# stockeh/swift

Hardware: AMD Instinct MI355X
Metric: 6h forecast steps/sec (members x ICs) on 128x256x69 ERA5 (higher is better)
Workload: dtype bf16

## Files before the change

### swift_amd/csrc/gemm.hip

```cpp
#include "common.h"

int g_persist_wgs = 256;

namespace {

template <typename OutT>
__device__ __forceinline__ float swiglu_out(float g, float u) {
    if constexpr (sizeof(OutT) == 4) return g / (1.0f + expf(-g)) * u;
    else return g * __builtin_amdgcn_rcpf(1.0f + __expf(-g)) * u;
}

constexpr int BM = 256;
constexpr int BN = 352;
constexpr int ROWB = 128;
constexpr int A_BYTES = BM * ROWB;
constexpr int B_BYTES = BN * ROWB;
constexpr int STAGE = A_BYTES + B_BYTES;
constexpr int LDS_BYTES = 2 * STAGE;
constexpr int NT = 512;
constexpr int A_PIECES = A_BYTES / 1024;
constexpr int B_PIECES = B_BYTES / 1024;
constexpr int MI = 4, NI = 11;

constexpr int EPI_QKNORM_TILED = 4;
// ... 241 lines not shown
    const int r16 = lane & 15;
    const int xoff = (wm * 64 + r16) * ROWB;
    const int woff = A_BYTES + (wn * 176 + r16) * ROWB;
    const int ch0 = (((lane >> 4) + 0) ^ (r16 >> 1)) * 16;
    const int ch1 = (((lane >> 4) + 4) ^ (r16 >> 1)) * 16;

    auto compute = [&](const char* s) {
#pragma unroll
        for (int ks = 0; ks < 2; ++ks) {
            const int ch = ks ? ch1 : ch0;
            uint4 xf[MI];
#pragma unroll
            for (int i = 0; i < MI; ++i) xf[i] = *reinterpret_cast<const uint4*>(s + xoff + i * 16 * ROWB + ch);
#pragma unroll
            for (int j = 0; j < NI; ++j) {
                const uint4 wf = *reinterpret_cast<const uint4*>(s + woff + j * 16 * ROWB + ch);
#pragma unroll
                for (int i = 0; i < MI; ++i) mma_chunk<T>(acc[i][j], wf, xf[i]);
            }
        }
    };

    const int nk = g.K / (ROWB / (int)sizeof(T));
    stage_load(stage0, 0);
    for (int kt = 0; kt < nk; kt += 2) {
        __builtin_amdgcn_s_waitcnt(0x0F70);
        __syncthreads();
        if (kt + 1 < nk) stage_load(stage1, kt + 1);
        compute(stage0);
        if (kt + 1 < nk) {
            __builtin_amdgcn_s_waitcnt(0x0F70);
            __syncthreads();
            if (kt + 2 < nk) stage_load(stage0, kt + 2);
            compute(stage1);
        }
    }

    if constexpr (EPI == SWIFTK_EPI_QKNORM || EPI == EPI_QKNORM_TILED)
        qknorm_tile<NI>(acc, lane, n0 + wn * 176, g.ep0, const_cast<float*>(g.ep1), m0 + wm * 64, g.M, g.N / 88);
    OutT* C = reinterpret_cast<OutT*>(g.C);
#pragma unroll
    for (int i = 0; i < MI; ++i) {
        const int m = m0 + wm * 64 + i * 16 + r16;
        if (m >= g.M) continue;
#pragma unroll
        for (int j = 0; j < NI; ++j) {
            const int nb = n0 + wn * 176 + j * 16 + 4 * (lane >> 4);
            if (nb >= g.N) continue;
            f32x4 v = acc[i][j];
            if constexpr (EPI == SWIFTK_EPI_BIAS_POS) {
                const float4 b = *reinterpret_cast<const float4*>(g.ep0 + nb);
                v[0] += b.x; v[1] += b.y; v[2] += b.z; v[3] += b.w;
                if (g.ep1) {
                    const float4 p = *reinterpret_cast<const float4*>(g.ep1 + (int64_t)(m % g.pos_rows) * g.N + nb);
                    v[0] += p.x; v[1] += p.y; v[2] += p.z; v[3] += p.w;
                }
            }
            if constexpr (EPI == SWIFTK_EPI_SWIGLU) {
                const float h0 = swiglu_out<OutT>(v[0], v[1]);
                const float h1 = swiglu_out<OutT>(v[2], v[3]);
                store2<OutT>(C + (int64_t)m * g.ldc + (nb >> 1), h0, h1);
            } else {
                store4<OutT>(C + (int64_t)m * g.ldc + nb, v[0], v[1], v[2], v[3]);
            }
        }
    }
}


struct TileIter {
    int ntm, ntn, gm;
    __device__ __forceinline__ void coords(int t, int& tm, int& tn) const {
        const int per = gm * ntn;
        const int grp = t / per, r = t - grp * per;
        const int rows = min(gm, ntm - grp * gm);
        tn = r / rows;
        tm = grp * gm + (r - tn * rows);
    }
};

template <typename T, typename OutT, int EPI, int NI, bool PPK, int SL = 0>
__global__ __launch_bounds__(NT) void gemm_kernel_p(GemmArgs g, int ntm, int gm) {
    constexpr bool SLE = (SL & 1) != 0, SLW = (SL & 2) != 0;
    static_assert(SL == 0 || (sizeof(T) == 2 && sizeof(OutT) == 2 && PPK && (EPI == SWIFTK_EPI_NONE || EPI == SWIFTK_EPI_SWIGLU)),
                  "the straight-line forms exist for the bf16 plain and SwiGLU epilogues of the ping-pong kernel only");
    constexpr int WT = 16 * NI;
    constexpr int BN = 2 * WT;
    constexpr int B_BYTES = BN * ROWB;
    constexpr int STAGE = A_BYTES + B_BYTES;
    constexpr int WP = B_BYTES / 1024;
    constexpr int HD = 8 * NI;
    constexpr bool PAIRED = EPI == SWIFTK_EPI_QKNORM_JVP || EPI == SWIFTK_EPI_SWIGLU_JVP;
    constexpr bool PP = PPK && sizeof(T) == 2;
    __shared__ __attribute__((aligned(16))) char smem[2 * STAGE];
    const int lane = threadIdx.x & 63;
    const int wv = __builtin_amdgcn_readfirstlane(threadIdx.x >> 6);
    const int wm = wv >> 1, wn = wv & 1;
    const TileIter it{ntm, g.ntn, gm};
    constexpr bool TAIL = EPI == EPI_NONE_TAIL;
    const int ksplit = TAIL || SLW ? 1 : g.ksplit;
    const int tail_from = TAIL ? g.tail_from : 0;
    const int ntiles = TAIL ? 2 * ntm * g.ntn - tail_from : ntm * g.ntn * ksplit;
    auto tile_of = [&](int item) {
        if constexpr (TAIL) return item < tail_from ? item : tail_from + ((item - tail_from) >> 1);
        else return item / ksplit;
    };
    auto split_of = [&](int item) {
        if constexpr (TAIL) return item < tail_from ? 0 : (item - tail_from) & 1;
        else return item % ksplit;
    };
    int vid;
    {
        const int nwg = gridDim.x, bid = blockIdx.x;
        const int q = nwg >> 3, r = nwg & 7, xcd = bid & 7;
        vid = (xcd < r ? xcd * (q + 1) : r * (q + 1) + (xcd - r) * q) + (bid >> 3);
    }
    const int stride = gridDim.x;
    if (vid >= ntiles) return;
    const uint32_t lds0 = (uint32_t)(uintptr_t)LDS_PTR(smem);

    const int prow = lane >> 3, pchunk = lane & 7;
    const uint32_t va_even = (uint32_t)(prow * g.lda_b) + 16u * (pchunk ^ ((prow >> 1) & 7));
    const uint32_t va_odd = (uint32_t)(prow * g.lda_b) + 16u * (pchunk ^ ((4 + (prow >> 1)) & 7));
    const uint32_t vb = (uint32_t)(prow * g.ldw_b) + 16u * (pchunk ^ ((4 * (wv & 1) + (prow >> 1)) & 7));
    [[maybe_unused]] const int tr2 = min(256 + wv * ((BN - 256 + 7) / 8) + min(lane, (BN - 256 + 7) / 8 - 1), BN - 1);
    [[maybe_unused]] int t_n0 = 0;
    const int nk_all = g.K / (ROWB / (int)sizeof(T));
    auto k_begin = [&](int item) {
        if constexpr (TAIL) return item >= tail_from && ((item - tail_from) & 1) ? nk_all >> 1 : 0;
        else return (int)((int64_t)(item % ksplit) * nk_all / ksplit);
    };
    auto k_end = [&](int item) {
        if constexpr (TAIL) return item >= tail_from && !((item - tail_from) & 1) ? nk_all >> 1 : nk_all;
        else return (int)((int64_t)(item % ksplit + 1) * nk_all / ksplit);
    };
    int tile = vid, kt = k_begin(vid);
    int w_grp = 0, w_tn = 0, w_rr = 0, s_grp = 0, s_tn = 0, s_rr = 0, n_tm = 0, n_tn = 0, c_tm = 0, c_tn = 0;
    if constexpr (SLW) {
        const int per = gm * g.ntn;
        w_grp = vid / per;
        int r = vid - w_grp * per;
        w_tn = r / gm;
        w_rr = r - w_tn * gm;
        s_grp = stride / per;
        r = stride - s_grp * per;
        s_tn = r / gm;
        s_rr = r - s_tn * gm;
    }
    auto walk_coords = [&](int& tm, int& tn) {
        const int rows = ntm - w_grp * gm;
        tm = w_grp * gm + w_rr;
        tn = w_tn;
        if (rows < gm) {
            const int r = w_tn * gm + w_rr;
            tn = r / rows;
            tm = w_grp * gm + (r - tn * rows);
        }
    };
    auto walk_step = [&] {
        w_rr += s_rr;
        int c = w_rr >= gm;
        w_rr -= c ? gm : 0;
        w_tn += s_tn + c;
        c = w_tn >= g.ntn;
        w_tn -= c ? g.ntn : 0;
        w_grp += s_grp + c;
    };
    auto src_coords = [&](int t, int& tm, int& tn) {
        if constexpr (SLW) { tm = n_tm; tn = n_tn; }
        else it.coords(tile_of(t), tm, tn);
    };
    const char* abase[4];
    const char* wbase[6];
    auto set_sources = [&](int t) {
        int tm, tn;
        it.coords(tile_of(t), tm, tn);
        t_n0 = tn * BN;
#pragma unroll
        for (int p = 0; p < 4; ++p) {
            int rb = tm * BM + (wv * 4 + p) * 8;
            if constexpr (PAIRED)
                rb = ((wv & 1) ? (g.M >> 1) : 0) + tm * (BM / 2) + (wv >> 1) * 32 + (p >> 1) * 16 + (p & 1) * 8;
            rb = rb < g.M ? rb : g.M - 8;
            abase[p] = g.A + (int64_t)rb * g.lda_b;
        }
#pragma unroll
        for (int i = 0; i < 6; ++i) {
            int rb = tn * BN + (wv + 8 * i) * 8;
            rb = rb < g.N ? rb : g.N - 8;
            if constexpr (sizeof(T) == 4 && EPI == SWIFTK_EPI_QKNORM)
                if (g.qk_only) rb += (rb / (2 * HD)) * HD;
            wbase[i] = g.W + (int64_t)rb * g.ldw_b;
        }
    };
    constexpr int JA = NI / 2, JB = NI - JA, JM = JA > JB ? JA : JB;
    const char* w0base[3];
    const char* w1base[3];
    auto w0row = [&](int i) { const int n = wv + 8 * i, h = n >= 2 * JA; return h * WT + (n - 2 * JA * h) * 8; };
    auto w1row = [&](int i) { const int n = wv + 8 * i, h = n >= 2 * JB; return h * WT + JA * 16 + (n - 2 * JB * h) * 8; };
    auto set_sources_aw1 = [&](int t) {
        int tm, tn;
        src_coords(t, tm, tn);
#pragma unroll
        for (int p = 0; p < 4; ++p) {
            int rb = tm * BM + (wv * 4 + p) * 8;
            if constexpr (PAIRED) rb = ((wv & 1) ? (g.M >> 1) : 0) + tm * (BM / 2) + (wv >> 1) * 32 + (p >> 1) * 16 + (p & 1) * 8;
            rb = rb < g.M ? rb : g.M - 8;
            abase[p] = g.A + (int64_t)rb * g.lda_b;
        }
#pragma unroll
        for (int i = 0; i < 3; ++i) {
            int rb = tn * BN + w1row(i);
            rb = rb < g.N ? rb : g.N - 8;
            w1base[i] = g.W + (int64_t)rb * g.ldw_b;
        }
    };
    auto set_sources_w0 = [&](int t) {
        int tm, tn;
        src_coords(t, tm, tn);
#pragma unroll
        for (int i = 0; i < 3; ++i) {
            int rb = tn * BN + w0row(i);
            rb = rb < g.N ? rb : g.N - 8;
            w0base[i] = g.W + (int64_t)rb * g.ldw_b;
        }
    };
    auto pp_a = [&](uint32_t sa, uint32_t koff, int p) {
        dma_piece_fast(sa + (wv * 4 + p) * 1024, abase[p], ((p & 1) ? va_odd : va_even) + koff);
    };
    auto pp_w0 = [&](uint32_t sa, uint32_t koff, int i) {
        if (wv + 8 * i < 4 * JA) dma_piece_fast(sa + A_BYTES + w0row(i) * ROWB, w0base[i], vb + koff);
    };
    auto pp_w1 = [&](uint32_t sa, uint32_t koff, int i) {
        if (wv + 8 * i < 4 * JB) dma_piece_fast(sa + A_BYTES + w1row(i) * ROWB, w1base[i], vb + koff);
    };
    auto issue_piece = [&](uint32_t sa, uint32_t koff, int p) {
        if (p < 4) {
            dma_piece_fast(sa + (wv * 4 + p) * 1024, abase[p], ((p & 1) ? va_odd : va_even) + koff);
        } else {
            const int i = p - 4;
            if (wv + 8 * i < WP) dma_piece_fast(sa + A_BYTES + (wv + 8 * i) * 1024, wbase[i], vb + koff);
        }
    };

    f32x4 acc[MI][NI];
#pragma unroll
    for (int i = 0; i < MI; ++i)
#pragma unroll
        for (int j = 0; j < NI; ++j) acc[i][j] = f32x4{0.f, 0.f, 0.f, 0.f};

    const int r16 = lane & 15;
    const int xoff = (wm * 64 + r16) * ROWB;
    const int woff = A_BYTES + (wn * WT + r16) * ROWB;
    const int ch0 = (((lane >> 4) + 0) ^ (r16 >> 1)) * 16;
    const int ch1 = (((lane >> 4) + 4) ^ (r16 >> 1)) * 16;

    int nk = k_end(tile);
    if constexpr (PP) {
        if constexpr (SLW) walk_coords(n_tm, n_tn);
        set_sources_aw1(tile);
        set_sources_w0(tile);
#pragma unroll
        for (int p = 0; p < 4; ++p) pp_a(lds0, (uint32_t)kt * ROWB, p);
#pragma unroll
        for (int i = 0; i < 3; ++i) pp_w0(lds0, (uint32_t)kt * ROWB, i);
#pragma unroll
        for (int i = 0; i < 3; ++i) pp_w1(lds0, (uint32_t)kt * ROWB, i);
    } else {
        set_sources(tile);
#pragma unroll
        for (int p = 0; p < 10; ++p) issue_piece(lds0, (uint32_t)kt * ROWB, p);
    }
    int par = 0;
    bool have_part = false;
    if (g.stagger != 0) {
        const int ph = g.stagger > 0 ? (((vid % gm) + (vid / gm)) & 7) : (int)(blockIdx.x & 7);
        const uint64_t t0 = __builtin_amdgcn_s_memrealtime();
        const uint64_t wait = (uint64_t)ph * (uint64_t)(g.stagger > 0 ? g.stagger : -g.stagger);
        while (__builtin_amdgcn_s_memrealtime() - t0 < wait) __builtin_amdgcn_s_sleep(16);
    }
    if (!PP && wv >= 4) __builtin_amdgcn_s_setprio(1);
    asm volatile("s_waitcnt vmcnt(0)" ::: "memory");
    const int grp = wv >> 2;
    bool first_kt = true;
#if SWIFTK_PP_STAMP
    unsigned long long* plog = nullptr;
    int pl_tile = 0, pl_kt = 0, pl_i = 0;
    if ((g.dbg & 64) && (wv & 3) == 0 && lane == 0 && (blockIdx.x & 31) == 0)
        plog = reinterpret_cast<unsigned long long*>(const_cast<float*>(g.ep1)) + ((blockIdx.x >> 5) * 2 + (wv >> 2)) * 20 * 16;
#define PP_STAMP() do { if (plog && pl_tile == 1 && pl_i < 16) plog[pl_kt * 16 + pl_i++] = __builtin_amdgcn_s_memtime(); } while (0)
#else
#define PP_STAMP() do {} while (0)
#endif
    for (;;) {
        if constexpr (PP) {
            if (first_kt) {
                __builtin_amdgcn_s_barrier();
                if (grp) __builtin_amdgcn_s_barrier();
            }
        } else {
            __builtin_amdgcn_s_barrier();
        }
        const char* s = smem + par * STAGE;
        const uint32_t fill = lds0 + (par ^ 1) * STAGE;
        const bool last_k = (kt + 1 == nk);
        const bool half = g.khalf && (kt + 1 == nk_all);
        uint32_t koff = (uint32_t)(kt + 1) * ROWB;
        if constexpr (PP) {
            const int ntile = tile + stride < ntiles ? tile + stride : tile;
            if (last_k) {
                if constexpr (SLW) {
                    walk_coords(c_tm, c_tn);
                    if (ntile != tile) walk_step();
                    walk_coords(n_tm, n_tn);
                }
                set_sources_aw1(ntile);
                set_sources_w0(ntile);
                koff = (uint32_t)k_begin(ntile) * ROWB;
            }
        } else
        if (last_k) {
            const int ntile = tile + stride;
            if (ntile < ntiles) set_sources(ntile);
            koff = (uint32_t)k_begin(ntile < ntiles ? ntile : tile) * ROWB;
// ... 286 lines not shown
                            const int j = jh + jj;
                            const int nb = n0 + wn * WT + j * 16 + 4 * g4;
                            const f32x4 v = acc[i][j];
                            acc[i][j] = f32x4{0.f, 0.f, 0.f, 0.f};
                            const uint4 hq = hb[gidx & 1][jj];
                            const uint32_t hw[4] = {hq.x, hq.y, hq.z, hq.w};
                            uint32_t o[4];
#pragma unroll
                            for (int e = 0; e < 4; ++e) {
                                const float gt = __uint_as_float(hw[e] << 16), up = __uint_as_float(hw[e] & 0xffff0000u);
                                const float sg = __builtin_amdgcn_rcpf(1.0f + __expf(-gt));
                                o[e] = pack_bf16(v[e] * up * (sg + gt * sg * (1.0f - sg)), v[e] * gt * sg);
                            }
                            if (m < g.M && nb < g.N)
                                *reinterpret_cast<uint4*>(C + (int64_t)m * g.ldc + 2 * nb) = make_uint4(o[0], o[1], o[2], o[3]);
                        }
                    }
                }
            } else
            if constexpr (EPI == SWIFTK_EPI_SWIGLU_BOTH) {
                constexpr int RS1 = WT * 2 + 16, RS2 = WT + 16;
                constexpr int CP1 = WT / 8, CP2 = WT / 16;
                __builtin_amdgcn_s_barrier();
                interior = (m0 + BM <= g.M) && (n0 + BN <= g.N);
                char* slab = const_cast<char*>(s) + wv * (16 * RS1);
                int elane = lane;
                asm volatile("" : "+v"(elane));
                const int g4 = elane >> 4;
                const int r16 = elane & 15;
                bf16_t* C2 = reinterpret_cast<bf16_t*>(const_cast<float*>(g.ep1));
                const int64_t ldc2 = g.pos_rows;
#pragma unroll
                for (int i = 0; i < MI; ++i) {
                    const int mrow0 = m0 + wm * 64 + i * 16;
#pragma unroll
                    for (int j = 0; j < NI; ++j) {
                        const f32x4 v = acc[i][j];
                        *reinterpret_cast<uint2*>(slab + r16 * RS1 + (j * 16 + 4 * g4) * 2) =
                            make_uint2(pack_bf16(v[0], v[1]), pack_bf16(v[2], v[3]));
                    }
                    __builtin_amdgcn_wave_barrier();
#pragma unroll
                    for (int t = 0; t < (16 * CP1 + 63) / 64; ++t) {
                        const int c = elane + 64 * t;
                        const int row = c / CP1, cc = c - row * CP1;
                        if (c < 16 * CP1) {
                            const uint4 q = *reinterpret_cast<const uint4*>(slab + row * RS1 + cc * 16);
                            const int m = mrow0 + row, n = n0 + wn * WT + cc * 8;
                            if (m < g.M && n < g.N) *reinterpret_cast<uint4*>(C + (int64_t)m * g.ldc + n) = q;
                        }
                    }
                    __builtin_amdgcn_wave_barrier();
#pragma unroll
                    for (int j = 0; j < NI; ++j) {
                        const f32x4 v = acc[i][j];
                        acc[i][j] = f32x4{0.f, 0.f, 0.f, 0.f};
                        const float h0 = v[0] * __builtin_amdgcn_rcpf(1.0f + __expf(-v[0])) * v[1];
                        const float h1 = v[2] * __builtin_amdgcn_rcpf(1.0f + __expf(-v[2])) * v[3];
                        *reinterpret_cast<uint32_t*>(slab + r16 * RS2 + (j * 8 + 2 * g4) * 2) = pack_bf16(h0, h1);
                    }
                    __builtin_amdgcn_wave_barrier();
#pragma unroll
                    for (int t = 0; t < (16 * CP2 + 63) / 64; ++t) {
                        const int c = elane + 64 * t;
                        const int row = c / CP2, cc = c - row * CP2;
                        if (c < 16 * CP2) {
                            const uint4 q = *reinterpret_cast<const uint4*>(slab + row * RS2 + cc * 16);
                            const int m = mrow0 + row, n = (n0 >> 1) + wn * (WT / 2) + cc * 8;
                            if (m < g.M && n < (g.N >> 1)) *reinterpret_cast<uint4*>(C2 + (int64_t)m * ldc2 + n) = q;
                        }
                    }
                    __builtin_amdgcn_wave_barrier();
                }
            } else
            if constexpr (sizeof(OutT) == 2 && EPI != SWIFTK_EPI_BIAS_POS) {
                constexpr bool SPLIT3 = EPI == SWIFTK_EPI_SWIGLU_SPLIT3;
                constexpr bool PAIROUT = EPI == EPI_BIAS_POS_PAIR;
                constexpr bool GLU = EPI == SWIFTK_EPI_SWIGLU || SPLIT3;
                constexpr int COLS = GLU ? WT / 2 : WT;
                constexpr int CPR = COLS / 8;
                constexpr int RSTR = COLS * 2 + 16;
                __builtin_amdgcn_s_barrier();
                interior = (m0 + BM <= g.M) && (n0 + BN <= g.N);
                char* slab = const_cast<char*>(s) + wv * (16 * RSTR);
                int elane = lane;
                asm volatile("" : "+v"(elane));
                const int g4 = elane >> 4;
                const int r16 = elane & 15;
                const int ncol0 = (GLU ? (n0 >> 1) : n0) + wn * COLS;
                const int nout = GLU ? (g.N >> 1) : g.N;
                uint32_t lo_pk[SPLIT3 || PAIROUT ? NI : 1];
                bool sl_done = false;
                if constexpr (SLE) {
                    if (interior) {
                        int el = lane;
                        asm volatile("" : "+v"(el));
                        const int sr16 = el & 15, sg4 = (el >> 4) & 3, l64 = el & 63;
                        constexpr int NCH = (16 * CPR + 63) / 64;
                        constexpr bool PART = (16 * CPR) % 64 != 0;
                        char* wr = slab + sr16 * RSTR + sg4 * (GLU ? 4 : 8);
                        const uint32_t ldcb = (uint32_t)g.ldc * 2u;
                        uint32_t ro[NCH], go[NCH];
#pragma unroll
                        for (int t = 0; t < NCH; ++t) {
                            const int c = l64 + 64 * t;
                            const int row = c / CPR, cc = c - row * CPR;
                            ro[t] = (uint32_t)(row * RSTR + cc * 16);
                            go[t] = (uint32_t)row * ldcb + (uint32_t)(cc * 16);
                        }
                        const bool part_on = l64 + 64 * (NCH - 1) < 16 * CPR;
                        char* cb = reinterpret_cast<char*>(C) + ((int64_t)(m0 + wm * 64) * g.ldc + ncol0) * 2;
#pragma unroll
                        for (int i = 0; i < MI; ++i) {
#pragma unroll
                            for (int j = 0; j < NI; ++j) {
                                const f32x4 v = acc[i][j];
                                acc[i][j] = f32x4{0.f, 0.f, 0.f, 0.f};
                                if constexpr (GLU) {
                                    const float h0 = v[0] * __builtin_amdgcn_rcpf(1.0f + __expf(-v[0])) * v[1];
                                    const float h1 = v[2] * __builtin_amdgcn_rcpf(1.0f + __expf(-v[2])) * v[3];
                                    *reinterpret_cast<uint32_t*>(wr + j * 16) = pack_bf16(h0, h1);
                                } else {
                                    *reinterpret_cast<uint2*>(wr + j * 32) = make_uint2(pack_bf16(v[0], v[1]), pack_bf16(v[2], v[3]));
                                }
                            }
                            __builtin_amdgcn_wave_barrier();
                            uint4 q[NCH];
#pragma unroll
                            for (int t = 0; t < NCH; ++t) q[t] = *reinterpret_cast<const uint4*>(slab + ro[t]);
#pragma unroll
                            for (int t = 0; t < NCH; ++t) {
                                if (!PART || t + 1 < NCH || part_on) store16_out_sbase(cb, go[t], q[t]);
                            }
                            __builtin_amdgcn_wave_barrier();
                            cb += (int64_t)g.ldc * 32;
                        }
                        sl_done = true;
                    }
                }
                if (!sl_done)
#pragma unroll
                for (int ii = 0; ii < MI; ++ii) {
                    const int i = EPI == SWIFTK_EPI_QKNORM_JVP ? ((ii & 1) ? ii >> 1 : 2 + (ii >> 1)) : ii;
#pragma unroll
                    for (int j = 0; j < NI; ++j) {
                        f32x4 v = acc[i][j];
                        if constexpr (EPI == SWIFTK_EPI_QKNORM_JVP) {
                            const bool first = 16 * j + 12 < 8 * NI ? true : (16 * j >= 8 * NI ? false : 16 * j + 4 * g4 < 8 * NI);
                            const float f = first ? qf[i & 1][0] : qf[i & 1][1];
                            if (i >= 2) {
                                const float fc = first ? qf[i & 1][2] : qf[i & 1][3];
                                const f32x4 pv = acc[i & 1][j];
#pragma unroll
                                for (int e = 0; e < 4; ++e) v[e] = fmaf(-fc, pv[e], f * v[e]);
                            } else {
                                v *= f;
                            }
                        }
                        acc[i][j] = f32x4{0.f, 0.f, 0.f, 0.f};
                        if constexpr (PAIROUT) {
                            const int nb = n0 + wn * WT + j * 16 + 4 * g4;
                            const int m = m0 + wm * 64 + i * 16 + r16;
                            if (m < g.M && nb < g.N) {
                                const float4 b = *reinterpret_cast<const float4*>(g.ep0 + nb);
                                v[0] += b.x; v[1] += b.y; v[2] += b.z; v[3] += b.w;
                                if (g.ep1) {
                                    const float4 pp = *reinterpret_cast<const float4*>(g.ep1 + (int64_t)(m % g.pos_rows) * g.N + nb);
                                    v[0] += pp.x; v[1] += pp.y; v[2] += pp.z; v[3] += pp.w;
                                }
                            }
                            const uint32_t h0 = pack_bf16(v[0], v[1]), h1 = pack_bf16(v[2], v[3]);
                            uint32_t lb = 0u;
                            lb = lo8_insert(v[0], __uint_as_float(h0 << 16), (h0 >> 7) & 0xFFu, 0, lb);
                            lb = lo8_insert(v[1], __uint_as_float(h0 & 0xffff0000u), (h0 >> 23) & 0xFFu, 1, lb);
                            lb = lo8_insert(v[2], __uint_as_float(h1 << 16), (h1 >> 7) & 0xFFu, 2, lb);
                            lb = lo8_insert(v[3], __uint_as_float(h1 & 0xffff0000u), (h1 >> 23) & 0xFFu, 3, lb);
                            lo_pk[j] = lb;
                            *reinterpret_cast<uint2*>(slab + r16 * RSTR + (j * 16 + 4 * g4) * 2) = make_uint2(h0, h1);
                        } else if constexpr (SPLIT3) {
                            const float h0 = swiglu_out<float>(v[0], v[1]), h1 = swiglu_out<float>(v[2], v[3]);
                            const uint32_t hp = pack_bf16(h0, h1);
                            lo_pk[j] = pack_bf16(h0 - __uint_as_float(hp << 16), h1 - __uint_as_float(hp & 0xffff0000u));
                            *reinterpret_cast<uint32_t*>(slab + r16 * RSTR + (j * 8 + 2 * g4) * 2) = hp;
                        } else if constexpr (EPI == SWIFTK_EPI_SWIGLU) {
                            const float h0 = v[0] * __builtin_amdgcn_rcpf(1.0f + __expf(-v[0])) * v[1];
                            const float h1 = v[2] * __builtin_amdgcn_rcpf(1.0f + __expf(-v[2])) * v[3];
                            *reinterpret_cast<uint32_t*>(slab + r16 * RSTR + (j * 8 + 2 * g4) * 2) = pack_bf16(h0, h1);
                        } else {
                            *reinterpret_cast<uint2*>(slab + r16 * RSTR + (j * 16 + 4 * g4) * 2) =
                                make_uint2(pack_bf16(v[0], v[1]), pack_bf16(v[2], v[3]));
                        }
                    }
                    __builtin_amdgcn_wave_barrier();
                    const int mrow0 = PAIRED ? (i >= 2 ? (g.M >> 1) : 0) + tm * (BM / 2) + wm * 32 + (i & 1) * 16 : m0 + wm * 64 + i * 16;
                    int tb = 0, try_ = 0, tx16 = 0, twin0 = 0;
                    if constexpr (EPI == EPI_QKNORM_TILED) {
                        {
                            const int ntok = g.t_gh * g.t_gw;
                            tb = mrow0 / ntok;
                            const int tt = mrow0 - tb * ntok, y = tt / g.t_gw;
                            tx16 = tt - y * g.t_gw;
                            try_ = y - g.t_sh;
                            try_ += try_ < 0 ? g.t_gh : 0;
                            twin0 = tb * ((g.t_gh >> 4) * (g.t_gw >> 4)) + (try_ >> 4) * (g.t_gw >> 4);
                        }
                    }
                    constexpr int NCH = (16 * CPR + 63) / 64;
#pragma unroll
                    for (int t = 0; t < NCH; ++t) {
                        const int c = elane + 64 * t;
                        const int row = c / CPR, cc = c - row * CPR;
                        if (c < 16 * CPR) {
                            const uint4 q = *reinterpret_cast<const uint4*>(slab + row * RSTR + cc * 16);
                            const int m = mrow0 + row, n = ncol0 + cc * 8;
                            int64_t dst = (int64_t)m * g.ldc + n;
                            if constexpr (EPI == EPI_QKNORM_TILED) {
                                {
                                    int rx = tx16 + row - g.t_sw;
                                    rx += rx < 0 ? g.t_gw : 0;
                                    const int hi = cc >= NI;
                                    const int tile_ = (twin0 + (rx >> 4)) * (3 * g.t_heads) + tn * 4 + wn * 2 + hi;
                                    dst = (int64_t)tile_ * (256 * HD) + ((((try_ & 15) << 4) | (rx & 15)) * HD + (cc - NI * hi) * 8);
                                }
                            }
                            if (m < g.M && n < nout) store16_out(C + dst, q);
                            if constexpr (SPLIT3) {
                                if (m < g.M && n < nout) store16_out(C + dst + 2 * (int64_t)g.pos_rows, q);
                            }
                        }
                    }
                    __builtin_amdgcn_wave_barrier();
                    if constexpr (SPLIT3) {
#pragma unroll
                        for (int j = 0; j < NI; ++j) *reinterpret_cast<uint32_t*>(slab + r16 * RSTR + (j * 8 + 2 * g4) * 2) = lo_pk[j];
                        __builtin_amdgcn_wave_barrier();
#pragma unroll
                        for (int t = 0; t < (16 * CPR + 63) / 64; ++t) {
                            const int c = elane + 64 * t;
                            const int row = c / CPR, cc = c - row * CPR;
                            if (c < 16 * CPR) {
                                const uint4 q = *reinterpret_cast<const uint4*>(slab + row * RSTR + cc * 16);
                                const int m = mrow0 + row, n = ncol0 + cc * 8;
                                if (m < g.M && n < nout) store16_out(C + (int64_t)m * g.ldc + n + g.pos_rows, q);
                            }
                        }
                        __builtin_amdgcn_wave_barrier();
                    }
                    if constexpr (PAIROUT) {
                        constexpr int RB = WT + 16, CB = WT / 16;
                        uint8_t* lo = reinterpret_cast<uint8_t*>(g.kscr);
#pragma unroll
                        for (int j = 0; j < NI; ++j) *reinterpret_cast<uint32_t*>(slab + r16 * RB + j * 16 + 4 * g4) = lo_pk[j];
                        __builtin_amdgcn_wave_barrier();
#pragma unroll
                        for (int t = 0; t < (16 * CB + 63) / 64; ++t) {
                            const int c = elane + 64 * t;
                            const int row = c / CB, cc = c - row * CB;
                            if (c < 16 * CB) {
                                const uint4 q = *reinterpret_cast<const uint4*>(slab + row * RB + cc * 16);
                                const int m = mrow0 + row, n = n0 + wn * WT + cc * 16;
                                if (m < g.M && n < g.N) store16_out(lo + (int64_t)m * g.c_split + n, q);
                            }
                        }
                        __builtin_amdgcn_wave_barrier();
                    }
                }
            } else if constexpr (EPI == SWIFTK_EPI_ACCUM) {
                constexpr int JH = 4, GPI = (NI + JH - 1) / JH, NG = MI * GPI;
                float4 buf[2][JH];
                auto load_group = [&](int gidx, float4 (&b)[JH]) {
                    const int i = gidx / GPI, jh = (gidx - i * GPI) * JH;
                    const int m = m0 + wm * 64 + i * 16 + r16;
#pragma unroll
                    for (int jj = 0; jj < JH; ++jj) {
                        const int nb = n0 + wn * WT + (jh + jj) * 16 + 4 * (lane >> 4);
                        b[jj] = make_float4(0.f, 0.f, 0.f, 0.f);
                        if (jh + jj < NI && m < g.M && nb < g.N) b[jj] = *reinterpret_cast<const float4*>(C + (int64_t)m * g.ldc + nb);
                    }
                };
                load_group(0, buf[0]);
#pragma unroll
                for (int gidx = 0; gidx < NG; ++gidx) {
                    if (gidx + 1 < NG) load_group(gidx + 1, buf[(gidx + 1) & 1]);
                    const int i = gidx / GPI, jh = (gidx - i * GPI) * JH;
                    const int m = m0 + wm * 64 + i * 16 + r16;
#pragma unroll
                    for (int jj = 0; jj < JH; ++jj) {
                        if (jh + jj < NI) {
                            const int j = jh + jj;
                            const int nb = n0 + wn * WT + j * 16 + 4 * (lane >> 4);
                            const f32x4 v = acc[i][j];
                            const float4 o = buf[gidx & 1][jj];
                            acc[i][j] = f32x4{0.f, 0.f, 0.f, 0.f};
                            if (m < g.M && nb < g.N) store4<OutT>(C + (int64_t)m * g.ldc + nb, v[0] + o.x, v[1] + o.y, v[2] + o.z, v[3] + o.w);
                        }
                    }
                }
            } else
#pragma unroll
            for (int i = 0; i < MI; ++i) {
                const int m = m0 + wm * 64 + i * 16 + r16;
#pragma unroll
                for (int j = 0; j < NI; ++j) {
                    const int nb = n0 + wn * WT + j * 16 + 4 * (lane >> 4);
                    f32x4 v = acc[i][j];
                    acc[i][j] = f32x4{0.f, 0.f, 0.f, 0.f};
                    if (m >= g.M || nb >= g.N) continue;
                    if constexpr (EPI == SWIFTK_EPI_BIAS_POS) {
                        const float4 b = *reinterpret_cast<const float4*>(g.ep0 + nb);
                        v[0] += b.x; v[1] += b.y; v[2] += b.z; v[3] += b.w;
                        if (g.ep1) {
                            const float4 pp =
                                *reinterpret_cast<const float4*>(g.ep1 + (int64_t)(m % g.pos_rows) * g.N + nb);
                            v[0] += pp.x; v[1] += pp.y; v[2] += pp.z; v[3] += pp.w;
                        }
                    }
                    if constexpr (EPI == SWIFTK_EPI_SWIGLU) {
                        const float h0 = swiglu_out<OutT>(v[0], v[1]);
                        const float h1 = swiglu_out<OutT>(v[2], v[3]);
                        store2<OutT>(C + (int64_t)m * g.ldc + (nb >> 1), h0, h1);
                    } else {
                        int nbo = nb;
                        if constexpr (sizeof(T) == 4 && EPI == SWIFTK_EPI_QKNORM)
                            if (g.qk_only) nbo += (nb / (2 * HD)) * HD;
                        store4<OutT>(C + (int64_t)m * g.ldc + nbo, v[0], v[1], v[2], v[3]);
                    }
                }
            }
        }
        tile += stride;
        if (tile >= ntiles) break;
        kt = k_begin(tile);
        nk = k_end(tile);
        if (interior) {
            constexpr int NSTORE = (EPI == EPI_BIAS_POS_PAIR ? 4 * ((16 * (WT / 16) + 63) / 64) : 0) + (EPI == SWIFTK_EPI_SWIGLU_SPLIT3 ? 12 : 4) *
                                       ((16 * ((EPI == SWIFTK_EPI_SWIGLU || EPI == SWIFTK_EPI_SWIGLU_SPLIT3 ? WT / 2 : WT) / 8) + 63) / 64) +
                                   (EPI == SWIFTK_EPI_SWIGLU_BOTH ? 4 * ((16 * (WT / 16) + 63) / 64) : 0);
            if constexpr (sizeof(OutT) == 2 && EPI != SWIFTK_EPI_BIAS_POS) asm volatile("s_waitcnt vmcnt(%0)" ::"n"(NSTORE) : "memory");
            else asm volatile("s_waitcnt vmcnt(0)" ::: "memory");
        } else {
            asm volatile("s_waitcnt vmcnt(0)" ::: "memory");
        }
    }
    asm volatile("s_waitcnt vmcnt(0)" ::: "memory");
}

int g_variant = 1;
int g_group_m = 8;
int g_dbg = 0;
int g_stagger_permille = 0;
int g_pp = 1;
int g_gemm_sl = 2;

inline bool pp_ok(const GemmArgs& g) { return g_pp > 0 && (g.K / 64) / g.ksplit >= 3; }

struct Prof {
    int epilogue = -1, N = 0;
    static constexpr int MAXE = 4096;
    hipEvent_t ev[2 * MAXE];
    int created = 0, used = 0;
} g_prof;

template <typename T, typename OutT, int EPI>
constexpr bool sl_capable = sizeof(T) == 2 && sizeof(OutT) == 2 && (EPI == SWIFTK_EPI_NONE || EPI == SWIFTK_EPI_SWIGLU);
int g_gemm_sl_seen = 0;

template <typename T, typename OutT, int EPI>
int launch_p11_pp(const GemmArgs& g, int grid, int ntm, hipStream_t st) {
    if constexpr (sl_capable<T, OutT, EPI>) {
        if ((g_gemm_sl & 1) && g.ldc >= (int64_t(1) << 27)) return SWIFTK_ESHAPE;
        const int sl = g_gemm_sl & (g.ksplit == 1 ? 3 : 1);
        g_gemm_sl_seen |= 1 << sl;
        switch (sl) {
            case 1: hipLaunchKernelGGL((gemm_kernel_p<T, OutT, EPI, 11, true, 1>), dim3(grid), dim3(NT), 0, st, g, ntm, g_group_m); return 0;
            case 2: hipLaunchKernelGGL((gemm_kernel_p<T, OutT, EPI, 11, true, 2>), dim3(grid), dim3(NT), 0, st, g, ntm, g_group_m); return 0;
            case 3: hipLaunchKernelGGL((gemm_kernel_p<T, OutT, EPI, 11, true, 3>), dim3(grid), dim3(NT), 0, st, g, ntm, g_group_m); return 0;
        }
    }
    hipLaunchKernelGGL((gemm_kernel_p<T, OutT, EPI, 11, true>), dim3(grid), dim3(NT), 0, st, g, ntm, g_group_m);
    return 0;
}

template <typename T, typename OutT, int EPI, bool W320, bool W384, bool PPK>
int launch_width(const GemmArgs& g, int grid, int ntm, hipStream_t st) {
    if constexpr (W320)
        if (g.ni == 10) {
            hipLaunchKernelGGL((gemm_kernel_p<T, OutT, EPI, 10, PPK>), dim3(grid), dim3(NT), 0, st, g, ntm, g_group_m);
            return 0;
        }
    if constexpr (W384)
        if (g.ni == 12) {
            hipLaunchKernelGGL((gemm_kernel_p<T, OutT, EPI, 12, PPK>), dim3(grid), dim3(NT), 0, st, g, ntm, g_group_m);
            return 0;
        }
    if constexpr (PPK) return launch_p11_pp<T, OutT, EPI>(g, grid, ntm, st);
    hipLaunchKernelGGL((gemm_kernel_p<T, OutT, EPI, 11, false>), dim3(grid), dim3(NT), 0, st, g, ntm, g_group_m);
    return 0;
}
template <typename T, typename OutT, int EPI, bool W320, bool W384>
int launch_p(const GemmArgs& g, int ntm, hipStream_t st) {
    const int ntiles = ntm * g.ntn * g.ksplit;
    const int grid = ntiles < g_persist_wgs ? ntiles : g_persist_wgs;
    if constexpr (sizeof(T) == 2)
        if (pp_ok(g)) return launch_width<T, OutT, EPI, W320, W384, true>(g, grid, ntm, st);
    return launch_width<T, OutT, EPI, W320, W384, false>(g, grid, ntm, st);
}

template <typename T, typename OutT, int EPI>
int launch(const GemmArgs& g, hipStream_t st) {
    auto kern = gemm_kernel<T, OutT, EPI>;
    const int ntm = (g.M + BM - 1) / BM;
    if (sizeof(T) == 4 && EPI != SWIFTK_EPI_QKNORM && g.ni != NI) return SWIFTK_ESHAPE;
    if (g.qk_only && (sizeof(T) != 4 || sizeof(OutT) != 4 || EPI != SWIFTK_EPI_QKNORM || g_variant == 0 || (g.M & 7) || (g.N & 7) || g.ep1))
        return SWIFTK_ESHAPE;
    const bool timed = swiftk_prof_begin(EPI, g.N, st);
    const bool wide_ok = sizeof(OutT) != 2 || (!((uintptr_t)g.C & 15) && !(g.ldc & 7) &&
                                               !(g.N & (EPI == SWIFTK_EPI_SWIGLU || EPI == SWIFTK_EPI_SWIGLU_BOTH ? 15 : 7)));
    if (g_variant == 0 || (g.M & 7) || (g.N & 7) || !wide_ok) {
        if (g.ksplit != 1 || g.t_gw || EPI == SWIFTK_EPI_ACCUM || EPI == SWIFTK_EPI_SWIGLU_BOTH || EPI == SWIFTK_EPI_SWIGLU_BWD)
            return SWIFTK_ESHAPE;
        if ((EPI == SWIFTK_EPI_QKNORM || EPI == EPI_QKNORM_TILED) && g.ni != NI) return SWIFTK_ESHAPE;
        GemmArgs g1 = g;
        g1.ntn = (g.N + BN - 1) / BN;
        hipLaunchKernelGGL(kern, dim3(ntm * g1.ntn), dim3(NT), 0, st, g1);
    } else {
        constexpr bool WIDE = sizeof(T) == 2 || EPI == SWIFTK_EPI_QKNORM;
        if (const int rc = launch_p<T, OutT, EPI, WIDE, WIDE>(g, ntm, st)) return rc;
    }
    if (timed) swiftk_prof_end(st);
    SWIFTK_CHECK_LAUNCH();
    return 0;
}

template <int EPI>
int launch_paired(const GemmArgs& g, hipStream_t st) {
    const int ntm = (g.M + BM - 1) / BM;
    constexpr bool W384 = EPI != EPI_BIAS_POS_PAIR;
    if (!W384 && g.ni == 12) return SWIFTK_ESHAPE;
    const bool timed = swiftk_prof_begin(EPI, g.N, st);
    if (const int rc = launch_p<bf16_t, bf16_t, EPI, true, W384>(g, ntm, st)) return rc;
    if (timed) swiftk_prof_end(st);
    SWIFTK_CHECK_LAUNCH();
    return 0;
}

template <typename T, typename OutT>
int dispatch_epi(int epi, const GemmArgs& g, hipStream_t st) {
    switch (epi) {
        case SWIFTK_EPI_NONE: return launch<T, OutT, SWIFTK_EPI_NONE>(g, st);
        case SWIFTK_EPI_BIAS_POS: return launch<T, OutT, SWIFTK_EPI_BIAS_POS>(g, st);
        case SWIFTK_EPI_SWIGLU: return launch<T, OutT, SWIFTK_EPI_SWIGLU>(g, st);
        case SWIFTK_EPI_SWIGLU_BWD:
            if constexpr (sizeof(OutT) == 2 && sizeof(T) == 2) return launch<T, OutT, SWIFTK_EPI_SWIGLU_BWD>(g, st);
            return SWIFTK_EINVAL;
        case SWIFTK_EPI_SWIGLU_BOTH:
            if constexpr (sizeof(OutT) == 2 && sizeof(T) == 2) return launch<T, OutT, SWIFTK_EPI_SWIGLU_BOTH>(g, st);
            return SWIFTK_EINVAL;
        case SWIFTK_EPI_ACCUM:
            if constexpr (sizeof(OutT) == 4) return launch<T, OutT, SWIFTK_EPI_ACCUM>(g, st);
            return SWIFTK_EINVAL;
        case SWIFTK_EPI_QKNORM:
            if constexpr (sizeof(OutT) == 2)
                if (g.t_gw) return launch<T, OutT, EPI_QKNORM_TILED>(g, st);
            return launch<T, OutT, SWIFTK_EPI_QKNORM>(g, st);
        case SWIFTK_EPI_SWIGLU_SPLIT3:
            if constexpr (sizeof(OutT) == 2 && sizeof(T) == 2) {
                if ((g.M & 7) || (g.N & 15) || ((uintptr_t)g.C & 15) || (g.ldc & 7) || (g.pos_rows & 7)) return SWIFTK_ESHAPE;
                return launch_paired<SWIFTK_EPI_SWIGLU_SPLIT3>(g, st);
            }
            return SWIFTK_EINVAL;
    }
    return SWIFTK_EINVAL;
}

}

bool swiftk_prof_begin(int kind, int n, hipStream_t st) {
    if (g_prof.epilogue != kind || (g_prof.N != 0 && g_prof.N != n) || g_prof.used >= Prof::MAXE) return false;
    while (g_prof.created <= g_prof.used) {
        if (hipEventCreate(&g_prof.ev[2 * g_prof.created]) != hipSuccess) return false;
        if (hipEventCreate(&g_prof.ev[2 * g_prof.created + 1]) != hipSuccess) return false;
        ++g_prof.created;
    }
    return hipEventRecord(g_prof.ev[2 * g_prof.used], st) == hipSuccess;
}

void swiftk_prof_end(hipStream_t st) {
    (void)hipEventRecord(g_prof.ev[2 * g_prof.used + 1], st);
    ++g_prof.used;
}

static const struct { int key; int* value; } g_tuning[] = {
    {0, &g_variant},          {1, &g_group_m},      {2, &g_persist_wgs},    {3, &g_dbg},           {4, &g_attn_dbg},
    {5, &g_fwd_tiled},        {6, &g_modnorm_nt},   {7, &g_stagger_permille}, {8, &g_fwd_fused},   {9, &g_attn_bwd_pipe},
    {11, &g_x3_exact},        {12, &g_fwd_pair},    {13, &g_f32_chunk_k},   {14, &g_fwd_splitk},   {15, &g_attn_bwd_fuse},
    {16, &g_modnorm_bwd_fused}, {17, &g_modnorm_jvp_rows}, {18, &g_x3_ffsplit}, {19, &g_fwd_pepair}, {20, &g_pp},
    {21, &g_attn_pp},         {22, &g_tn_pp},       {23, &g_fwd_rownorm},   {24, &g_rownorm_dbg},  {25, &g_zero_memset},
    {26, &g_x3_normsplit},    {27, &g_x3_qkonly},   {28, &g_x3_attnpv},     {29, &g_fwd_tail},     {30, &g_attn_sl},
    {31, &g_gemm_sl},         {32, &g_gemm_sl_seen},
};

static int* tuning_value(int key) {
    for (const auto& row : g_tuning)
        if (row.key == key) return row.value;
    return nullptr;
}

extern "C" int swiftk_set_tuning(int key, int value) {
    switch (key) {
        case 1:
        case 2: value = value > 0 ? value : 1; break;
        case 30:
        case 31: value &= 3; break;
        case 32: value = 0; break;
        case 25: g_zero_memset = value; return (value & 4) ? swiftk_zero_check_enable() : 0;
    }
    int* const p = tuning_value(key);
    if (!p) return SWIFTK_EINVAL;
    *p = value;
    return 0;
}

extern "C" int swiftk_get_tuning(int key) {
    const int* const p = tuning_value(key);
    return p ? *p : SWIFTK_EINVAL;
}

extern "C" int swiftk_profile_gemm(int epilogue, int64_t N) {
    g_prof.epilogue = epilogue;
    g_prof.N = (int)N;
    g_prof.used = 0;
    return 0;
}

extern "C" int swiftk_profile_collect(double* total_ms, int64_t* launches) {
    if (!total_ms || !launches) return SWIFTK_EINVAL;
    double tot = 0.0;
    for (int i = 0; i < g_prof.used; ++i) {
        if (hipEventSynchronize(g_prof.ev[2 * i + 1]) != hipSuccess) return SWIFTK_EINVAL;
        float ms = 0.f;
        if (hipEventElapsedTime(&ms, g_prof.ev[2 * i], g_prof.ev[2 * i + 1]) != hipSuccess) return SWIFTK_EINVAL;
        tot += ms;
    }
    *total_ms = tot;
    *launches = g_prof.used;
    g_prof.used = 0;
    return 0;
}

extern "C" int64_t swiftk_gemm_k_pad(int dtype, int64_t k) {
    const int64_t g = dtype == SWIFTK_BF16 ? 64 : 32;
    return (k + g - 1) / g * g;
}

static int gemm_impl(const void* A, int64_t lda, const void* W, int64_t ldw, void* C, int64_t ldc, int64_t M, int64_t N,
                     int64_t K, int dtype, int out_dtype, int epilogue, const float* ep0, const float* ep1, int64_t pos_rows,
                     int ksplit, int64_t c_split, void* stream, const int* tiling = nullptr, float* kscr = nullptr,
                     int kchunk = 0, int64_t* tail_rows_from = nullptr) {
    if (!A || !W || !C || M <= 0 || N <= 0 || K <= 0 || ksplit < 1) return SWIFTK_EINVAL;
    if (tail_rows_from && (ksplit != 1 || dtype != SWIFTK_BF16 || out_dtype != SWIFTK_BF16 || epilogue != SWIFTK_EPI_NONE || c_split < M * ldc))
        return SWIFTK_EINVAL;
    if (ksplit > 1 && ((out_dtype != SWIFTK_F32 && !(out_dtype == SWIFTK_BF16 && dtype == SWIFTK_BF16)) || epilogue != SWIFTK_EPI_NONE || c_split < M * ldc))
        return SWIFTK_EINVAL;
    if (epilogue == SWIFTK_EPI_ACCUM && out_dtype != SWIFTK_F32) return SWIFTK_EINVAL;
    if (epilogue == SWIFTK_EPI_SWIGLU_BWD && (out_dtype != SWIFTK_BF16 || !ep1 || ((uintptr_t)ep1 & 15) || pos_rows < 2 * N || pos_rows % 8 ||
                                              ldc < 2 * N || ldc % 8 || ((uintptr_t)C & 15)))
        return SWIFTK_EINVAL;
    if (epilogue == SWIFTK_EPI_SWIGLU_SPLIT3 && (dtype != SWIFTK_BF16 || out_dtype != SWIFTK_BF16 || pos_rows < N / 2 || ldc < 2 * pos_rows + N / 2))
        return SWIFTK_EINVAL;
    if (epilogue == SWIFTK_EPI_SWIGLU_BOTH && (out_dtype != SWIFTK_BF16 || !ep1 || ((uintptr_t)ep1 & 15) || pos_rows < N / 2 || pos_rows % 8 || N % 16))
        return SWIFTK_EINVAL;
    if (dtype != SWIFTK_F32 && dtype != SWIFTK_BF16) return SWIFTK_EINVAL;
    if (out_dtype != SWIFTK_F32 && out_dtype != dtype) return SWIFTK_EINVAL;
    const int es = dtype == SWIFTK_BF16 ? 2 : 4, os = out_dtype == SWIFTK_BF16 ? 2 : 4;
    const int tile_k = ROWB / es;
    int khalf = 0;
    if (K % tile_k == tile_k / 2 && lda >= K + tile_k / 2 && ldw >= K + tile_k / 2) {
        khalf = 1;
        K += tile_k / 2;
    }
    if (K % tile_k != 0 || N % 4 != 0) return SWIFTK_ESHAPE;
    if (M > (1 << 30) || N > (1 << 30) || K > (1 << 30)) return SWIFTK_ESHAPE;
    if (lda < K || ldw < K) return SWIFTK_ESHAPE;
    if (ksplit > K / tile_k) return SWIFTK_ESHAPE;
    const int ovec = (epilogue == SWIFTK_EPI_SWIGLU || epilogue == SWIFTK_EPI_SWIGLU_SPLIT3 ? 2 : 4) * os;
    if (((uintptr_t)A & 15) || ((uintptr_t)W & 15) || (lda * es) % 16 || (ldw * es) % 16) return SWIFTK_EALIGN;
    if (((uintptr_t)C % ovec) || (ldc * os) % ovec) return SWIFTK_EALIGN;
    int ni = 11;
    int qk_only = 0;
    if (epilogue == SWIFTK_EPI_QKNORM && pos_rows < 0) {
        qk_only = 1;
        pos_rows = -pos_rows;
        if (dtype != SWIFTK_F32 || out_dtype != SWIFTK_F32 || N % (4 * pos_rows) != 0) return SWIFTK_ESHAPE;
    }
    if (epilogue == SWIFTK_EPI_QKNORM) {
        const int64_t hd = pos_rows > 0 ? pos_rows : 88;
// ... 192 lines not shown
```

Before: 385.7.

## Add straight-line epilogue for bias+pos pair GEMM and narrow-N fp32 walk path

Measured after the change: 386.9, median of 6. Within noise of the previous version (+0.3%).

```diff
diff --git a/swift_amd/csrc/gemm.hip b/swift_amd/csrc/gemm.hip
--- a/swift_amd/csrc/gemm.hip
+++ b/swift_amd/csrc/gemm.hip
@@ -347,8 +347,10 @@
 template <typename T, typename OutT, int EPI, int NI, bool PPK, int SL = 0>
 __global__ __launch_bounds__(NT) void gemm_kernel_p(GemmArgs g, int ntm, int gm) {
     constexpr bool SLE = (SL & 1) != 0, SLW = (SL & 2) != 0;
-    static_assert(SL == 0 || (sizeof(T) == 2 && sizeof(OutT) == 2 && PPK && (EPI == SWIFTK_EPI_NONE || EPI == SWIFTK_EPI_SWIGLU)),
-                  "the straight-line forms exist for the bf16 plain and SwiGLU epilogues of the ping-pong kernel only");
+    static_assert(SL == 0 || (sizeof(T) == 2 && PPK &&
+                              (sizeof(OutT) == 2 ? (EPI == SWIFTK_EPI_NONE || EPI == SWIFTK_EPI_SWIGLU || EPI == EPI_BIAS_POS_PAIR)
+                                                 : (EPI == SWIFTK_EPI_NONE && !SLE))),
+                  "the straight-line forms exist for the bf16 plain, SwiGLU and pair epilogues of the ping-pong kernel (fp32 output: the walk) only");
     constexpr int WT = 16 * NI;
     constexpr int BN = 2 * WT;
     constexpr int B_BYTES = BN * ROWB;
@@ -388,6 +390,16 @@
     const uint32_t va_even = (uint32_t)(prow * g.lda_b) + 16u * (pchunk ^ ((prow >> 1) & 7));
     const uint32_t va_odd = (uint32_t)(prow * g.lda_b) + 16u * (pchunk ^ ((4 + (prow >> 1)) & 7));
     const uint32_t vb = (uint32_t)(prow * g.ldw_b) + 16u * (pchunk ^ ((4 * (wv & 1) + (prow >> 1)) & 7));
+    constexpr bool NEDGE = NI == 9;
+    uint32_t vb_edge = vb;
+    int wedge = 0;
+    auto straddles = [&](int rb) { return rb < g.N && rb + 8 > g.N; };
+    if constexpr (NEDGE) {
+        const int nrem = g.N & 7;
+        const int pr = nrem && prow >= nrem ? nrem - 1 : prow;
+        vb_edge = (uint32_t)(pr * g.ldw_b) + 16u * (pchunk ^ ((4 * (wv & 1) + (prow >> 1)) & 7));
+    }
+    auto vb_of = [&](int bit) { return NEDGE && ((wedge >> bit) & 1) ? vb_edge : vb; };
     [[maybe_unused]] const int tr2 = min(256 + wv * ((BN - 256 + 7) / 8) + min(lane, (BN - 256 + 7) / 8 - 1), BN - 1);
     [[maybe_unused]] int t_n0 = 0;
     const int nk_all = g.K / (ROWB / (int)sizeof(T));
@@ -463,6 +475,12 @@
     const char* w1base[3];
     auto w0row = [&](int i) { const int n = wv + 8 * i, h = n >= 2 * JA; return h * WT + (n - 2 * JA * h) * 8; };
     auto w1row = [&](int i) { const int n = wv + 8 * i, h = n >= 2 * JB; return h * WT + JA * 16 + (n - 2 * JB * h) * 8; };
+    if constexpr (NEDGE) {
+#pragma unroll
+        for (int i = 0; i < 3; ++i) wedge |= (straddles(w0row(i)) ? 1 << i : 0) | (straddles(w1row(i)) ? 8 << i : 0);
+#pragma unroll
+        for (int i = 0; i < 6; ++i) wedge |= straddles((wv + 8 * i) * 8) ? 256 << i : 0;
+    }
     auto set_sources_aw1 = [&](int t) {
         int tm, tn;
         src_coords(t, tm, tn);
@@ -494,17 +512,17 @@
         dma_piece_fast(sa + (wv * 4 + p) * 1024, abase[p], ((p & 1) ? va_odd : va_even) + koff);
     };
     auto pp_w0 = [&](uint32_t sa, uint32_t koff, int i) {
-        if (wv + 8 * i < 4 * JA) dma_piece_fast(sa + A_BYTES + w0row(i) * ROWB, w0base[i], vb + koff);
+        if (wv + 8 * i < 4 * JA) dma_piece_fast(sa + A_BYTES + w0row(i) * ROWB, w0base[i], vb_of(i) + koff);
     };
     auto pp_w1 = [&](uint32_t sa, uint32_t koff, int i) {
-        if (wv + 8 * i < 4 * JB) dma_piece_fast(sa + A_BYTES + w1row(i) * ROWB, w1base[i], vb + koff);
+        if (wv + 8 * i < 4 * JB) dma_piece_fast(sa + A_BYTES + w1row(i) * ROWB, w1base[i], vb_of(3 + i) + koff);
     };
     auto issue_piece = [&](uint32_t sa, uint32_t koff, int p) {
         if (p < 4) {
             dma_piece_fast(sa + (wv * 4 + p) * 1024, abase[p], ((p & 1) ? va_odd : va_even) + koff);
         } else {
             const int i = p - 4;
-            if (wv + 8 * i < WP) dma_piece_fast(sa + A_BYTES + (wv + 8 * i) * 1024, wbase[i], vb + koff);
+            if (wv + 8 * i < WP) dma_piece_fast(sa + A_BYTES + (wv + 8 * i) * 1024, wbase[i], vb_of(8 + i) + koff);
         }
     };
 
@@ -957,7 +975,10 @@
                 constexpr int RSTR = COLS * 2 + 16;
                 __builtin_amdgcn_s_barrier();
                 interior = (m0 + BM <= g.M) && (n0 + BN <= g.N);
-                char* slab = const_cast<char*>(s) + wv * (16 * RSTR);
+                constexpr int PRB = WT + 16;
+                constexpr int PSLAB = SLE && PAIROUT ? ((16 * (RSTR + PRB) + 1023) & ~1023) : 16 * RSTR;
+                static_assert(8 * PSLAB <= STAGE, "the slabs overlay one stage");
+                char* slab = const_cast<char*>(s) + wv * PSLAB;
                 int elane = lane;
                 asm volatile("" : "+v"(elane));
                 const int g4 = elane >> 4;
@@ -966,7 +987,7 @@
                 const int nout = GLU ? (g.N >> 1) : g.N;
                 uint32_t lo_pk[SPLIT3 || PAIROUT ? NI : 1];
                 bool sl_done = false;
-                if constexpr (SLE) {
+                if constexpr (SLE && !PAIROUT) {
                     if (interior) {
                         int el = lane;
                         asm volatile("" : "+v"(el));
@@ -1013,6 +1034,104 @@
                         sl_done = true;
                     }
                 }
+                if constexpr (SLE && PAIROUT) {
+                    if (interior && g.ep1 && (g.pos_rows & (BM - 1)) == 0) {
+                        int el = lane;
+                        asm volatile("" : "+v"(el));
+                        const int sr16 = el & 15, sg4 = (el >> 4) & 3;
+                        constexpr int RB = PRB;
+                        char* hs = slab;
+                        char* ls = hs + 16 * RSTR;
+                        char* wr_h = hs + sr16 * RSTR + sg4 * 8;
+                        char* wr_l = ls + sr16 * RB + sg4 * 4;
+                        const int mw = m0 + wm * 64, ncw = n0 + wn * WT;
+                        const int pm = m0 % g.pos_rows + wm * 64;
+                        const char* pb = reinterpret_cast<const char*>(g.ep1 + ((int64_t)pm * g.N + ncw));
+                        const uint32_t prow_b = (uint32_t)g.N * 4u;
+                        const uint32_t poff = (uint32_t)sr16 * prow_b + (uint32_t)sg4 * 16u;
+                        const char* bb = reinterpret_cast<const char*>(g.ep0 + ncw) + sg4 * 16;
+                        constexpr int JH = 4, GPI = (NI + JH - 1) / JH, NG = MI * GPI;
+                        float4 pbuf[2][JH];
+                        auto load_group = [&](int gidx, float4 (&b)[JH]) {
+                            const int i = gidx / GPI, jh = (gidx - i * GPI) * JH;
+                            const char* pbi = pb + (int64_t)(16 * i) * prow_b;
+#pragma unroll
+                            for (int jj = 0; jj < JH; ++jj)
+                                if (jh + jj < NI) b[jj] = *reinterpret_cast<const float4*>(pbi + poff + (jh + jj) * 64);
+                        };
+                        load_group(0, pbuf[0]);
+#pragma unroll
+                        for (int jh = 0; jh < NI; jh += JH) {
+                            float4 b[JH];
+                            __builtin_amdgcn_sched_barrier(0);
+#pragma unroll
+                            for (int jj = 0; jj < JH; ++jj)
+                                if (jh + jj < NI) b[jj] = *reinterpret_cast<const float4*>(bb + (jh + jj) * 64);
+#pragma unroll
+                            for (int jj = 0; jj < JH; ++jj)
+                                if (jh + jj < NI) {
+#pragma unroll
+                                    for (int i = 0; i < MI; ++i) {
+                                        f32x4 v = acc[i][jh + jj];
+                                        v[0] += b[jj].x; v[1] += b[jj].y; v[2] += b[jj].z; v[3] += b[jj].w;
+                                        asm volatile("" : "+v"(v));
+                                        acc[i][jh + jj] = v;
+                                    }
+                                }
+                        }
+                        const int hr = (el >> 3) & 7, hq = el & 7, lr = (el >> 2) & 15, lq = el & 3;
+                        const uint32_t ldcb = (uint32_t)g.ldc * 2u, ldlb = (uint32_t)g.c_split;
+                        const char* rd_h = hs + hr * RSTR + hq * 16;
+                        const char* rd_l = ls + lr * RB + lq * 16;
+                        const uint32_t go_h = (uint32_t)hr * ldcb + (uint32_t)hq * 16u, go_l = (uint32_t)lr * ldlb + (uint32_t)lq * 16u;
+                        char* cb = reinterpret_cast<char*>(C) + ((int64_t)mw * g.ldc + ncw) * 2;
+                        char* lb_ = reinterpret_cast<char*>(g.kscr) + ((int64_t)mw * g.c_split + ncw);
+#pragma unroll
+                        for (int gidx = 0; gidx < NG; ++gidx) {
+                            __builtin_amdgcn_sched_barrier(0);
+                            if (gidx + 1 < NG) load_group(gidx + 1, pbuf[(gidx + 1) & 1]);
+                            __builtin_amdgcn_sched_barrier(0);
+                            const int i = gidx / GPI, jh = (gidx - i * GPI) * JH;
+#pragma unroll
+                            for (int jj = 0; jj < JH; ++jj) {
+                                if (jh + jj < NI) {
+                                    const int j = jh + jj;
+                                    const float4 pp = pbuf[gidx & 1][jj];
+                                    f32x4 v = acc[i][j];
+                                    v[0] += pp.x; v[1] += pp.y; v[2] += pp.z; v[3] += pp.w;
+                                    const uint32_t h0 = pack_bf16(v[0], v[1]), h1 = pack_bf16(v[2], v[3]);
+                                    uint32_t lb = 0u;
+                                    lb = lo8_insert(v[0], __uint_as_float(h0 << 16), (h0 >> 7) & 0xFFu, 0, lb);
+                                    lb = lo8_insert(v[1], __uint_as_float(h0 & 0xffff0000u), (h0 >> 23) & 0xFFu, 1, lb);
+                                    lb = lo8_insert(v[2], __uint_as_float(h1 << 16), (h1 >> 7) & 0xFFu, 2, lb);
+                                    lb = lo8_insert(v[3], __uint_as_float(h1 & 0xffff0000u), (h1 >> 23) & 0xFFu, 3, lb);
+                                    *reinterpret_cast<uint2*>(wr_h + j * 32) = make_uint2(h0, h1);
+                                    *reinterpret_cast<uint32_t*>(wr_l + j * 16) = lb;
+                                }
+                            }
+                            if (jh + JH >= NI) {
+                                __builtin_amdgcn_wave_barrier();
+                                char* cbi = cb + (int64_t)(16 * i) * ldcb;
+                                char* lbi = lb_ + (int64_t)(16 * i) * ldlb;
+#pragma unroll
+                                for (int h = 0; h < 2; ++h) {
+#pragma unroll
+                                    for (int t = 0; t < (CPR + 7) / 8; ++t)
+                                        if (8 * t + 8 <= CPR || hq + 8 * t < CPR)
+                                            *reinterpret_cast<uint4*>(cbi + (int64_t)(8 * h) * ldcb + go_h + t * 128) =
+                                                *reinterpret_cast<const uint4*>(rd_h + h * 8 * RSTR + t * 128);
+                                    __builtin_amdgcn_sched_barrier(0);
+                                }
+#pragma unroll
+                                for (int t = 0; t < (NI + 3) / 4; ++t)
+                                    if (4 * t + 4 <= NI || lq + 4 * t < NI)
+                                        *reinterpret_cast<uint4*>(lbi + go_l + t * 64) = *reinterpret_cast<const uint4*>(rd_l + t * 64);
+                                __builtin_amdgcn_wave_barrier();
+                            }
+                        }
+                        sl_done = true;
+                    }
+                }
                 if (!sl_done)
 #pragma unroll
                 for (int ii = 0; ii < MI; ++ii) {
@@ -1032,7 +1151,7 @@
                                 v *= f;
                             }
                         }
-                        acc[i][j] = f32x4{0.f, 0.f, 0.f, 0.f};
+                        if constexpr (!(SLE && PAIROUT)) acc[i][j] = f32x4{0.f, 0.f, 0.f, 0.f};
                         if constexpr (PAIROUT) {
                             const int nb = n0 + wn * WT + j * 16 + 4 * g4;
                             const int m = m0 + wm * 64 + i * 16 + r16;
@@ -1050,7 +1169,8 @@
                             lb = lo8_insert(v[1], __uint_as_float(h0 & 0xffff0000u), (h0 >> 23) & 0xFFu, 1, lb);
                             lb = lo8_insert(v[2], __uint_as_float(h1 << 16), (h1 >> 7) & 0xFFu, 2, lb);
                             lb = lo8_insert(v[3], __uint_as_float(h1 & 0xffff0000u), (h1 >> 23) & 0xFFu, 3, lb);
-                            lo_pk[j] = lb;
+                            if constexpr (SLE) *reinterpret_cast<uint32_t*>(slab + 16 * RSTR + r16 * PRB + j * 16 + 4 * g4) = lb;
+                            else lo_pk[j] = lb;
                             *reinterpret_cast<uint2*>(slab + r16 * RSTR + (j * 16 + 4 * g4) * 2) = make_uint2(h0, h1);
                         } else if constexpr (SPLIT3) {
                             const float h0 = swiglu_out<float>(v[0], v[1]), h1 = swiglu_out<float>(v[2], v[3]);
@@ -1124,21 +1244,30 @@
                     if constexpr (PAIROUT) {
                         constexpr int RB = WT + 16, CB = WT / 16;
                         uint8_t* lo = reinterpret_cast<uint8_t*>(g.kscr);
-#pragma unroll
-                        for (int j = 0; j < NI; ++j) *reinterpret_cast<uint32_t*>(slab + r16 * RB + j * 16 + 4 * g4) = lo_pk[j];
-                        __builtin_amdgcn_wave_barrier();
+                        const char* lslab = slab + (SLE ? 16 * RSTR : 0);
+                        if constexpr (!SLE) {
+#pragma unroll
+                            for (int j = 0; j < NI; ++j) *reinterpret_cast<uint32_t*>(slab + r16 * RB + j * 16 + 4 * g4) = lo_pk[j];
+                            __builtin_amdgcn_wave_barrier();
+                        }
 #pragma unroll
                         for (int t = 0; t < (16 * CB + 63) / 64; ++t) {
                             const int c = elane + 64 * t;
                             const int row = c / CB, cc = c - row * CB;
                             if (c < 16 * CB) {
-                                const uint4 q = *reinterpret_cast<const uint4*>(slab + row * RB + cc * 16);
+                                const uint4 q = *reinterpret_cast<const uint4*>(lslab + row * RB + cc * 16);
                                 const int m = mrow0 + row, n = n0 + wn * WT + cc * 16;
                                 if (m < g.M && n < g.N) store16_out(lo + (int64_t)m * g.c_split + n, q);
                             }
                         }
                         __builtin_amdgcn_wave_barrier();
                     }
+                }
+                if constexpr (SLE && PAIROUT) {
+#pragma unroll
+                    for (int i = 0; i < MI; ++i)
+#pragma unroll
+                        for (int j = 0; j < NI; ++j) acc[i][j] = f32x4{0.f, 0.f, 0.f, 0.f};
                 }
             } else if constexpr (EPI == SWIFTK_EPI_ACCUM) {
                 constexpr int JH = 4, GPI = (NI + JH - 1) / JH, NG = MI * GPI;
@@ -1226,6 +1355,7 @@
 int g_stagger_permille = 0;
 int g_pp = 1;
 int g_gemm_sl = 2;
+int g_gemm_ph = 3;
 
 inline bool pp_ok(const GemmArgs& g) { return g_pp > 0 && (g.K / 64) / g.ksplit >= 3; }
 
@@ -1242,6 +1372,15 @@
 
 template <typename T, typename OutT, int EPI>
 int launch_p11_pp(const GemmArgs& g, int grid, int ntm, hipStream_t st) {
+    if constexpr (EPI == EPI_BIAS_POS_PAIR) {
+        if ((g_gemm_ph & 1) && g.ksplit == 1) {
+            if (g.ldc >= (int64_t(1) << 27) || g.c_split >= (int64_t(1) << 27) || g.N >= (1 << 26)) return SWIFTK_ESHAPE;
+            g_gemm_sl_seen |= 1 << 3;
+            hipLaunchKernelGGL((gemm_kernel_p<T, OutT, EPI, 11, true, 3>), dim3(grid), dim3(NT), 0, st, g, ntm, g_group_m);
+            return 0;
+        }
+        g_gemm_sl_seen |= 1;
+    }
     if constexpr (sl_capable<T, OutT, EPI>) {
         if ((g_gemm_sl & 1) && g.ldc >= (int64_t(1) << 27)) return SWIFTK_ESHAPE;
         const int sl = g_gemm_sl & (g.ksplit == 1 ? 3 : 1);
@@ -1291,6 +1430,25 @@
     const bool timed = swiftk_prof_begin(EPI, g.N, st);
     const bool wide_ok = sizeof(OutT) != 2 || (!((uintptr_t)g.C & 15) && !(g.ldc & 7) &&
                                                !(g.N & (EPI == SWIFTK_EPI_SWIGLU || EPI == SWIFTK_EPI_SWIGLU_BOTH ? 15 : 7)));
+    if constexpr (sizeof(T) == 2 && sizeof(OutT) == 4 && EPI == SWIFTK_EPI_NONE) {
+        if ((g_gemm_ph & 2) && g_variant != 0 && g.N <= 288 && g.N >= 8 && g.M >= BM && !(g.M & 7) && g.ksplit == 1 && !g.t_gw) {
+            GemmArgs g9 = g;
+            g9.ni = 9;
+            g9.ntn = 1;
+            const int grid = ntm < g_persist_wgs ? ntm : g_persist_wgs;
+            if (pp_ok(g9)) {
+                g_gemm_sl_seen |= 1 << 4;
+                hipLaunchKernelGGL((gemm_kernel_p<T, OutT, EPI, 9, true, 2>), dim3(grid), dim3(NT), 0, st, g9, ntm, g_group_m);
+            } else {
+                g_gemm_sl_seen |= 1 << 6;
+                hipLaunchKernelGGL((gemm_kernel_p<T, OutT, EPI, 9, false>), dim3(grid), dim3(NT), 0, st, g9, ntm, g_group_m);
+            }
+            if (timed) swiftk_prof_end(st);
+            SWIFTK_CHECK_LAUNCH();
+            return 0;
+        }
+        if (g_variant == 0 || (g.M & 7) || (g.N & 7)) g_gemm_sl_seen |= 1 << 5;
+    }
     if (g_variant == 0 || (g.M & 7) || (g.N & 7) || !wide_ok) {
         if (g.ksplit != 1 || g.t_gw || EPI == SWIFTK_EPI_ACCUM || EPI == SWIFTK_EPI_SWIGLU_BOTH || EPI == SWIFTK_EPI_SWIGLU_BWD)
             return SWIFTK_ESHAPE;
@@ -1372,7 +1530,7 @@
     {16, &g_modnorm_bwd_fused}, {17, &g_modnorm_jvp_rows}, {18, &g_x3_ffsplit}, {19, &g_fwd_pepair}, {20, &g_pp},
     {21, &g_attn_pp},         {22, &g_tn_pp},       {23, &g_fwd_rownorm},   {24, &g_rownorm_dbg},  {25, &g_zero_memset},
     {26, &g_x3_normsplit},    {27, &g_x3_qkonly},   {28, &g_x3_attnpv},     {29, &g_fwd_tail},     {30, &g_attn_sl},
-    {31, &g_gemm_sl},         {32, &g_gemm_sl_seen},
+    {31, &g_gemm_sl},         {32, &g_gemm_sl_seen}, {33, &g_gemm_ph},
 };
 
 static int* tuning_value(int key) {
@@ -1386,7 +1544,8 @@
         case 1:
         case 2: value = value > 0 ? value : 1; break;
         case 30:
-        case 31: value &= 3; break;
+        case 31:
+        case 33: value &= 3; break;
         case 32: value = 0; break;
         case 25: g_zero_memset = value; return (value & 4) ? swiftk_zero_check_enable() : 0;
     }
```
